# davidmilligan/MLVFS

Measured on AMD Instinct MI355X. Metric: Mpix/s, 3584x1320 14-bit unpack+badpix+cs5x5+stripes (fused, stream resident in HBM), higher is better.
Workload: dtype u16/int32

## Files before the change

### mlvfs_amd/csrc/k_frame_dev.h

```cpp
#pragma once
#include "clip.h"
#include <cstdlib>
#include <map>
#include <mutex>
#include <vector>
#include <algorithm>
#include <cstdio>
#include <type_traits>

typedef short mlv_pk16 __attribute__((ext_vector_type(2)));
__device__ __forceinline__ int mlv_min_(int a, int b) { return min(a, b); }
__device__ __forceinline__ int mlv_max_(int a, int b) { return max(a, b); }
__device__ __forceinline__ mlv_pk16 mlv_min_(mlv_pk16 a, mlv_pk16 b) { return __builtin_elementwise_min(a, b); }
__device__ __forceinline__ mlv_pk16 mlv_max_(mlv_pk16 a, mlv_pk16 b) { return __builtin_elementwise_max(a, b); }
#define MLV_NET_FN __device__ __forceinline__
#define mlv_mn(a, b) mlv_min_((a), (b))
#define mlv_mx(a, b) mlv_max_((a), (b))
#include "median_nets.h"


namespace mlv {

constexpr int TCW = FRAME_TCW;
constexpr int TCH = FRAME_TCH;
// ... 861 lines not shown
    return p;
}


template <int BPP>
__device__ __forceinline__ void item_tile_offsets(const ItemLane &L, int l_row, int w, uint32_t &pre_a, uint32_t &pre_b)
{
    constexpr uint32_t GB = (uint32_t)BPP;
    const uint32_t pitch = (uint32_t)(w >> 3) * GB;
    const uint32_t rowoff = __umul24((uint32_t)(2 * l_row), pitch) + 16u;
    pre_a = rowoff + ((uint32_t)((L.xoff_a >> 3) * (int)GB) & L.amask);
    pre_b = rowoff + ((uint32_t)((L.xoff_b >> 3) * (int)GB) & L.amask) + L.boff;
}
template <int BPP, int VEC, class LANE>
__device__ __forceinline__ void issue_tile_rows_pre(uint32_t (&r0)[4], uint32_t (&r1)[4], const uint8_t *frame, unsigned bytes, uint32_t pre_a, uint32_t pre_b,
                                                    LANE lane_of, int w, int h, int tx0, int ty0, int new0)
{
    constexpr uint32_t GB = (uint32_t)BPP;
    const uint32_t pitch = (uint32_t)(w >> 3) * GB;
    const int ybase = ty0 - 2 * HC + 2 * new0;
    uint32_t oa0, ob0, oa1, ob1, S = 0;
    if (VEC != 2 && tx0 >= 8 && tx0 + 2 * TCW + 8 <= w && ybase + 2 * TCH <= h) {
        S = (uint32_t)ybase * pitch + (uint32_t)(tx0 >> 3) * GB - 16u;
        oa0 = pre_a;
        ob0 = pre_b;
        oa1 = oa0 + pitch;
        ob1 = ob0 + pitch;
    } else {
        int l_row;
        const ItemLane L = lane_of(l_row);
        const int y = ybase + 2 * l_row;
        const int gmax = (w >> 3) - 1, g0 = tx0 >> 3;
        const uint32_t ga = __umul24((uint32_t)min(g0 + (L.xoff_a >> 3), gmax), GB);
        const uint32_t gb = __umul24((uint32_t)max(min(g0 + (L.xoff_b >> 3), gmax), 0), GB);
        const uint32_t row0 = __umul24((uint32_t)min(y, h - 1), pitch), row1 = __umul24((uint32_t)min(y + 1, h - 1), pitch);
        oa0 = (row0 + ga) & L.amask; ob0 = ((row0 + gb) & L.amask) + L.boff;
        oa1 = (row1 + ga) & L.amask; ob1 = ((row1 + gb) & L.amask) + L.boff;
        asm volatile("" : "+v"(oa0), "+v"(ob0));
    }
    const mlv_i32x4 rs = frame_rsrc(frame + S, bytes - S);
    const mlv_u32x2 a0 = mlv_rbl_x2(rs, (int)oa0, 0, AUX_DEFAULT), b0 = mlv_rbl_x2(rs, (int)ob0, 0, AUX_DEFAULT);
    const mlv_u32x2 a1 = mlv_rbl_x2(rs, (int)oa1, 0, AUX_DEFAULT), b1 = mlv_rbl_x2(rs, (int)ob1, 0, AUX_DEFAULT);
    r0[0] = a0.x; r0[1] = a0.y; r0[2] = b0.x; r0[3] = b0.y;
    r1[0] = a1.x; r1[1] = a1.y; r1[2] = b1.x; r1[3] = b1.y;
}
template <int BPP, int VEC>
__device__ __forceinline__ void issue_tile_rows(uint32_t (&r0)[4], uint32_t (&r1)[4], const uint8_t *frame, unsigned bytes, const ItemLane &L, int l_row,
                                                int w, int h, int tx0, int ty0, int new0)
{
    uint32_t pre_a, pre_b;
    item_tile_offsets<BPP>(L, l_row, w, pre_a, pre_b);
    issue_tile_rows_pre<BPP, VEC>(r0, r1, frame, bytes, pre_a, pre_b, [&](int &row) { row = l_row; return L; }, w, h, tx0, ty0, new0);
}

struct OutArgs {
    const uint2 *e2d;
    uint8_t *dst;
    size_t dst_stride;
    int stripes, coef_pk, coef_fast, white;
    int co[8];
};
__device__ __forceinline__ OutArgs out_args(KArgs kt)
{
    OutArgs o;
    o.e2d = kt->e2d; o.dst = kt->dst; o.dst_stride = kt->dst_stride;
    o.stripes = kt->stripes; o.coef_pk = kt->coef_pk; o.coef_fast = kt->coef_fast; o.white = kt->white;
#pragma unroll
    for (int i = 0; i < 8; i++) o.co[i] = kt->coef[i];
    return o;
}

__device__ __forceinline__ void put_rb(uint32_t &top, uint32_t &bot, uint32_t ur, uint32_t ub, unsigned long long m)
{
    asm("s_mov_b64 vcc, %4\n\t"
        "v_cndmask_b32_sdwa %0, %0, %2, vcc dst_sel:WORD_0 dst_unused:UNUSED_PRESERVE src0_sel:WORD_0 src1_sel:WORD_0\n\t"
        "v_cndmask_b32_sdwa %1, %1, %3, vcc dst_sel:WORD_1 dst_unused:UNUSED_PRESERVE src0_sel:WORD_1 src1_sel:WORD_0"
        : "+v"(top), "+v"(bot) : "v"(ur), "v"(ub), "s"(m) : "vcc");
}
__device__ __forceinline__ unsigned long long lanes_gt(int a, int b) { return __builtin_amdgcn_sicmp(a, b, 38); }
__device__ __forceinline__ unsigned long long lanes_ge(int a, int b) { return __builtin_amdgcn_sicmp(a, b, 39); }
__device__ __forceinline__ unsigned long long lanes_lt(int a, int b) { return __builtin_amdgcn_sicmp(a, b, 40); }

struct NoSmem {};
__device__ __forceinline__ bool smoothed_low(const int (&er)[STRIP], const int (&eb)[STRIP])
{
    const int lo = min(min(min(min(er[0], er[1]), er[2]), min(er[3], eb[0])), min(min(eb[1], eb[2]), eb[3]));
    return __any(lo < 7 * MLV_EV_RES);
}
template <int METHOD, bool PACKED, bool VECST, bool CLAMP, bool XM, bool ANYSTRIPES, bool BRIGHT, class SM, bool RAWREG = false>
__device__ __forceinline__ void strip_output_t(const SM &sm, const OutArgs &oa, int w, int h, int black, int f, int tx0, int ty0, int jj, int kk,
                                               unsigned long long msmooth, const int (&gev)[STRIP], int gev_off, const int (&er)[STRIP], const int (&eb)[STRIP], bool store,
                                               uint32_t *rtop = nullptr, uint32_t *rbot = nullptr)
{
    const int y = ty0 + 2 * jj, x = tx0 + 2 * STRIP * kk;
    uint32_t top[STRIP], bot[STRIP];
    auto read_raw = [&]() {
        if constexpr (RAWREG) {
#pragma unroll
            for (int c = 0; c < STRIP; c++) { top[c] = rtop[c]; bot[c] = rbot[c]; }
        } else {
            const uint4 v0 = *(const uint4 *)&sm.raw[2 * jj][2 * STRIP * kk];
            const uint4 v1 = *(const uint4 *)&sm.raw[2 * jj + 1][2 * STRIP * kk];
            top[0] = v0.x; top[1] = v0.y; top[2] = v0.z; top[3] = v0.w;
            bot[0] = v1.x; bot[1] = v1.y; bot[2] = v1.z; bot[3] = v1.w;
        }
    };
    if (METHOD == 0) read_raw();
    if (METHOD != 0) {
        const mlv_i32x4 rs_e2d = table_rsrc(oa.e2d, 8, E2D_RECORDS_EXT);
        int ur[STRIP], ub[STRIP], cr[STRIP], cb[STRIP];
        mlv_tab_u32x2 dr2[STRIP], db2[STRIP];
#pragma unroll
        for (int c = 0; c < STRIP; c++) {
            cr[c] = CLAMP ? min(max(er[c], 0), MLV_EV_MAX) : er[c];
            cb[c] = CLAMP ? min(max(eb[c], 0), MLV_EV_MAX) : eb[c];
            dr2[c] = mlv_sbl_x2(rs_e2d, cr[c] >> 5, 0, 0, AUX_DEFAULT);
            db2[c] = mlv_sbl_x2(rs_e2d, cb[c] >> 5, 0, 0, AUX_DEFAULT);
        }
        read_raw();
        asm volatile("" :: "v"(dr2[0]), "v"(dr2[1]), "v"(dr2[2]), "v"(dr2[3]), "v"(db2[0]), "v"(db2[1]), "v"(db2[2]), "v"(db2[3]));
#pragma unroll
        for (int c = 0; c < STRIP; c++) {
            ur[c] = (int)(__builtin_popcount(bfe_low_bits(dr2[c].y, (uint32_t)cr[c])) + dr2[c].x);
            ub[c] = (int)(__builtin_popcount(bfe_low_bits(db2[c].y, (uint32_t)cb[c])) + db2[c].x);
        }
#pragma unroll
        for (int c = 0; c < STRIP; c++) {
            unsigned long long okm = msmooth;
            if (!BRIGHT) okm &= lanes_ge((int)((uint32_t)gev[c] - (uint32_t)gev_off), 2 * MLV_EV_RES) & lanes_gt(er[c], MLV_EV_RES) & lanes_gt(eb[c], MLV_EV_RES);
            if (XM) okm &= lanes_ge(x + 2 * c, 4) & lanes_lt(x + 2 * c, w - 4);
            put_rb(top[c], bot[c], (uint32_t)ur[c], (uint32_t)ub[c], okm);
        }
    }
    if (oa.stripes) {
        const int black16 = (int)(uint16_t)black, white16 = (int)(uint16_t)oa.white;
        if (!ANYSTRIPES) stripe_strip_pk<CLAMP>(top, bot, oa.co, black16, white16);
        else if (PACKED && oa.coef_pk) stripe_strip_pk<true>(top, bot, oa.co, black16, white16);
        else if (oa.coef_fast) stripe_strip<true>(top, bot, oa.co, black16, white16);
        else stripe_strip<false>(top, bot, oa.co, black16, white16);
    }
    if constexpr (RAWREG) {
#pragma unroll
        for (int c = 0; c < STRIP; c++) { rtop[c] = top[c]; rbot[c] = bot[c]; }
    }
    if (store && y < h) {
        if (VECST) {
            if (x < w) {
                const uint32_t T = ((uint32_t)ty0 * (uint32_t)w + (uint32_t)tx0) * 2u;
                const mlv_i32x4 rs_out = frame_rsrc(oa.dst + (size_t)f * oa.dst_stride + T, (uint32_t)w * (uint32_t)h * 2u - T);
                const uint32_t vo = (__umul24((uint32_t)(2 * jj), (uint32_t)w) + 2 * STRIP * (uint32_t)kk) * 2u;
                const mlv_u32x4 vt = { top[0], top[1], top[2], top[3] }, vb = { bot[0], bot[1], bot[2], bot[3] };
                mlv_rbs_x4(vt, rs_out, (int)vo, 0, 2);
                if (y + 1 < h) mlv_rbs_x4(vb, rs_out, (int)vo, w * 2, 2);
            }
        } else {
            uint16_t *out = (uint16_t *)(oa.dst + (size_t)f * oa.dst_stride);
#pragma unroll 1
            for (int c = 0; c < STRIP; c++) {
                const int xc = x + 2 * c;
                if (xc < w) out[(size_t)y * w + xc] = (uint16_t)top[c];
                if (xc + 1 < w) out[(size_t)y * w + xc + 1] = (uint16_t)(top[c] >> 16);
                if (y + 1 < h) {
                    if (xc < w) out[(size_t)(y + 1) * w + xc] = (uint16_t)bot[c];
                    if (xc + 1 < w) out[(size_t)(y + 1) * w + xc + 1] = (uint16_t)(bot[c] >> 16);
                }
            }
        }
    }
}

template <int METHOD, bool PACKED, bool VECST, class SM>
__device__ __forceinline__ void strip_output(const SM &sm, const OutArgs &oa, int w, int h, int black, int f, int tx0, int ty0, int jj, int kk,
                                             unsigned long long msmooth, const int (&gev)[STRIP], int gev_off, const int (&er)[STRIP], const int (&eb)[STRIP], bool low_any, bool bright,
                                             bool store)
{
    const bool xm = tx0 < 4 || tx0 + 2 * TCW > w - 4;
    if (METHOD != 0 && !low_any && oa.stripes && smoothed_low(er, eb)) { low_any = true; bright = false; }
    if (oa.stripes && !(PACKED && oa.coef_pk)) {
        strip_output_t<METHOD, PACKED, VECST, true, true, true, false, SM>(sm, oa, w, h, black, f, tx0, ty0, jj, kk, msmooth, gev, gev_off, er, eb, store);
    } else if (low_any) {
// ... 35 lines not shown
```

### mlvfs_amd/csrc/k_frame_p.hip

```cpp
#include "frame_plan.h"
#include "k_stream_dev.h"

namespace mlv {

constexpr int P_WAIT_MIN = 1, P_WAIT_MAX = 15;
template <bool SPREAD_>
struct __align__(16) SmemP {
    static constexpr bool SPREAD = SPREAD_;
    uint16_t raw[2 * RH][2 * TCW];
    uint32_t pk[PH][PW];
    int ge[RH][TCW];
    uint16_t t16[MLV_T16_N + (SPREAD_ ? 64 : 0)];
    uint32_t has_patch[PMAP_WORDS];
    uint32_t xchg[3][XCHG_WORDS];
    int unc[2];
    int low[2];
    int dim[2];
    int next_tile, next_end;
    int walk[5];
    int2 carry_at[256];
    uint4 carry_spare;
};

struct PGroup {
    mlv_pk16 s[4][5];
    mlv_pk16 p0[10], p1[10];
    mlv_pk16 q[6];
};
struct PNext { mlv_pk16 s0[5], s2[5], p0[10], q[6]; };

__device__ __forceinline__ mlv_pk16 as_pk(uint32_t v) { return __builtin_bit_cast(mlv_pk16, v); }
__device__ __forceinline__ uint32_t as_u(mlv_pk16 v) { return __builtin_bit_cast(uint32_t, v); }

__device__ __forceinline__ void pchain_group(const uint32_t (*pk)[PW], int row_top, int col_left, PGroup &g)
{
    mlv_pk16 col[4][5];
#pragma unroll
    for (int r = 0; r < 5; r++) {
        const uint4 v = *(const uint4 *)&pk[row_top + r][col_left];
        col[0][r] = as_pk(v.x); col[1][r] = as_pk(v.y); col[2][r] = as_pk(v.z); col[3][r] = as_pk(v.w);
    }
#pragma unroll
    for (int c = 0; c < 4; c++) mlv_sort5(col[c], g.s[c]);
    mlv_merge55(g.s[0], g.s[1], g.p0);
    mlv_merge55(g.s[2], g.s[3], g.p1);
}
__device__ __forceinline__ void pchain_fetch_lists(const PGroup &g, PNext &n)
{
#pragma unroll
    for (int i = 0; i < 5; i++) { n.s0[i] = dpp_next(g.s[0][i]); n.s2[i] = dpp_next(g.s[2][i]); }
#pragma unroll
    for (int i = 0; i < 10; i++) n.p0[i] = dpp_next(g.p0[i]);
}
__device__ __forceinline__ void pchain_fetch_window(const PGroup &g, PNext &n)
{
#pragma unroll
    for (int i = 0; i < 6; i++) n.q[i] = dpp_next(g.q[i]);
}
__device__ __forceinline__ void pchain_publish(const PGroup &g, uint32_t *x)
{
    uint4 *o = (uint4 *)x;
    o[0] = make_uint4(as_u(g.s[0][0]), as_u(g.s[0][1]), as_u(g.s[0][2]), as_u(g.s[0][3]));
    o[1] = make_uint4(as_u(g.s[0][4]), as_u(g.s[2][0]), as_u(g.s[2][1]), as_u(g.s[2][2]));
    o[2] = make_uint4(as_u(g.s[2][3]), as_u(g.s[2][4]), as_u(g.p0[0]), as_u(g.p0[1]));
    o[3] = make_uint4(as_u(g.p0[2]), as_u(g.p0[3]), as_u(g.p0[4]), as_u(g.p0[5]));
    o[4] = make_uint4(as_u(g.p0[6]), as_u(g.p0[7]), as_u(g.p0[8]), as_u(g.p0[9]));
    o[5] = make_uint4(as_u(g.q[0]), as_u(g.q[1]), as_u(g.q[2]), as_u(g.q[3]));
    *(uint2 *)&o[6] = make_uint2(as_u(g.q[4]), as_u(g.q[5]));
}
__device__ __forceinline__ void pchain_collect_lists(const uint32_t *x, PNext &n)
{
    const uint4 *o = (const uint4 *)x;
    const uint4 a0 = o[0], a1 = o[1], a2 = o[2], a3 = o[3], a4 = o[4];
    n.s0[0] = as_pk(a0.x); n.s0[1] = as_pk(a0.y); n.s0[2] = as_pk(a0.z); n.s0[3] = as_pk(a0.w); n.s0[4] = as_pk(a1.x);
    n.s2[0] = as_pk(a1.y); n.s2[1] = as_pk(a1.z); n.s2[2] = as_pk(a1.w); n.s2[3] = as_pk(a2.x); n.s2[4] = as_pk(a2.y);
    n.p0[0] = as_pk(a2.z); n.p0[1] = as_pk(a2.w); n.p0[2] = as_pk(a3.x); n.p0[3] = as_pk(a3.y); n.p0[4] = as_pk(a3.z);
    n.p0[5] = as_pk(a3.w); n.p0[6] = as_pk(a4.x); n.p0[7] = as_pk(a4.y); n.p0[8] = as_pk(a4.z); n.p0[9] = as_pk(a4.w);
}
__device__ __forceinline__ void pchain_collect_window(const uint32_t *x, PNext &n)
{
    const uint4 a5 = *(const uint4 *)(x + 20);
    const uint2 a6 = *(const uint2 *)(x + 24);
    n.q[0] = as_pk(a5.x); n.q[1] = as_pk(a5.y); n.q[2] = as_pk(a5.z); n.q[3] = as_pk(a5.w); n.q[4] = as_pk(a6.x); n.q[5] = as_pk(a6.y);
}
__device__ __forceinline__ void pchain_finish(const PGroup &g, const PNext &n, mlv_pk16 (&o)[STRIP])
{
    mlv_pk16 q1[6], t[1];
    mlv_quad_mid6(g.p1, n.p0, q1);
    mlv_final6of11(g.q, n.s0, t);  o[0] = t[0];
    mlv_final6of11(q1, g.s[1], t); o[1] = t[0];
    mlv_final6of11(q1, n.s2, t);   o[2] = t[0];
    mlv_final6of11(n.q, g.s[3], t); o[3] = t[0];
}
__device__ __forceinline__ bool pk_uncertain(const mlv_pk16 (&o)[STRIP])
{
    typedef unsigned short upk16 __attribute__((ext_vector_type(2)));
    const upk16 off = { 32769, 32769 }, two = { 2, 2 };
    upk16 m = __builtin_bit_cast(upk16, o[0]) + off;
#pragma unroll
    for (int c = 1; c < STRIP; c++) m = __builtin_elementwise_min(m, (upk16)(__builtin_bit_cast(upk16, o[c]) + off));
    return __builtin_bit_cast(uint32_t, __builtin_elementwise_min(m, two)) != 0x00020002u;
}

__device__ __forceinline__ uint32_t add3_u32(uint32_t a, uint32_t b, uint32_t c)
{
    uint32_t r;
    asm("v_add3_u32 %0, %1, %2, %3" : "=v"(r) : "v"(a), "v"(b), "v"(c));
    return r;
}
template <int NC, bool SPREAD>
__device__ __forceinline__ void cell_multi_pk_fast(const uint32_t *p0, const uint32_t *p1, int black, const uint16_t *t, int ref_r, int ref_b,
                                                   int (&ge)[NC], uint32_t (&pk)[NC])
{
    uint32_t fb[4 * NC], tv[4 * NC];
    const float fmagic = 8388608.0f + (float)black;
#pragma unroll
    for (int c = 0; c < NC; c++) {
        const uint32_t px[4] = { p0[2 * c], p0[2 * c + 1], p1[2 * c], p1[2 * c + 1] };
#pragma unroll
        for (int i = 0; i < 4; i++) fb[4 * c + i] = __float_as_uint(__uint_as_float(px[i] | 0x4B000000u) - fmagic);
    }
#pragma unroll
    for (int i = 0; i < 4 * NC; i++) tv[i] = *(const uint16_t *)((const char *)t + t16_offset<SPREAD>(fb[i]));
    uint32_t exr[NC], exb[NC], exg[NC];
#pragma unroll
    for (int c = 0; c < NC; c++) { exr[c] = fb[4 * c] >> 8; exb[c] = fb[4 * c + 3] >> 8; exg[c] = (fb[4 * c + 1] + fb[4 * c + 2]) >> 8; }
#pragma unroll
    for (int c = 0; c < NC; c += 2) {
        asm volatile("" :: "v"(exr[c]), "v"(exb[c]), "v"(exg[c]), "v"(exr[c + 1]), "v"(exb[c + 1]), "v"(exg[c + 1]));
    }
#pragma unroll
    for (int i = 0; i < 4 * NC; i += 8) {
        asm volatile("" :: "v"(tv[i]), "v"(tv[i + 1]), "v"(tv[i + 2]), "v"(tv[i + 3]), "v"(tv[i + 4]), "v"(tv[i + 5]), "v"(tv[i + 6]), "v"(tv[i + 7]));
    }
    uint32_t nref_r = 0u - (uint32_t)ref_r, nref_b = 0u - (uint32_t)ref_b;
    asm("" : "+v"(nref_r), "+v"(nref_b));
#pragma unroll
    for (int c = 0; c < NC; c++) {
        const uint32_t gb = add3_u32(exg[c], tv[4 * c + 1], tv[4 * c + 2]) >> 1;
        ge[c] = (int)(gb - (127u << 15));
        uint32_t ngr = nref_r - gb, ngb = nref_b - gb;
        pk[c] = as_u(__builtin_amdgcn_cvt_pk_i16((int)add3_u32(exr[c], tv[4 * c + 0], ngr), (int)add3_u32(exb[c], tv[4 * c + 3], ngb)));
    }
}

template <int NC>
__device__ __forceinline__ void cell_multi_pk_tab(const uint32_t *p0, const uint32_t *p1, uint32_t koff, const int *tab, int ref_r, int ref_b,
                                                  int (&ge)[NC], uint32_t (&pk)[NC])
{
    uint32_t ev[4 * NC];
#pragma unroll
    for (int c = 0; c < NC; c++) {
        const uint32_t px[4] = { p0[2 * c], p0[2 * c + 1], p1[2 * c], p1[2 * c + 1] };
#pragma unroll
        for (int i = 0; i < 4; i++) ev[4 * c + i] = *(const uint32_t *)((const char *)tab + ((px[i] << 2) + koff));
    }
#pragma unroll
    for (int i = 0; i < 4 * NC; i += 8) {
        asm volatile("" :: "v"(ev[i]), "v"(ev[i + 1]), "v"(ev[i + 2]), "v"(ev[i + 3]), "v"(ev[i + 4]), "v"(ev[i + 5]), "v"(ev[i + 6]), "v"(ev[i + 7]));
    }
    uint32_t nref_r = 1u - (uint32_t)ref_r, nref_b = 1u - (uint32_t)ref_b;
#pragma unroll
    for (int c = 0; c < NC; c++) {
        const uint32_t gb = (ev[4 * c + 1] + ev[4 * c + 2]) >> 1;
        ge[c] = (int)gb;
        const uint32_t ng = ~gb;
        pk[c] = as_u(__builtin_amdgcn_cvt_pk_i16((int)add3_u32(ev[4 * c + 0], nref_r, ng), (int)add3_u32(ev[4 * c + 3], nref_b, ng)));
    }
}
template <int NC>
__device__ __forceinline__ void cell_multi_pk_tab_dark(const uint32_t *p0, const uint32_t *p1, uint32_t koff, const int *tab, int ref_r, int ref_b,
                                                       int (&ge)[NC], uint32_t (&pk)[NC])
{
    int ev[4 * NC];
#pragma unroll
    for (int c = 0; c < NC; c++) {
        const uint32_t px[4] = { p0[2 * c], p0[2 * c + 1], p1[2 * c], p1[2 * c + 1] };
#pragma unroll
        for (int i = 0; i < 4; i++) ev[4 * c + i] = *(const int *)((const char *)tab + max((int)((px[i] << 2) + koff), 0));
    }
#pragma unroll
    for (int i = 0; i < 4 * NC; i += 8) {
        asm volatile("" :: "v"(ev[i]), "v"(ev[i + 1]), "v"(ev[i + 2]), "v"(ev[i + 3]), "v"(ev[i + 4]), "v"(ev[i + 5]), "v"(ev[i + 6]), "v"(ev[i + 7]));
    }
// ... 413 lines not shown
    const int plane = min(max(lane - 1, 0), PARK_LANES - 1);
    const bool parks = lane >= 1 && lane <= PARK_LANES;
    for (;;) {
        const int task = stream_draw(tickets, lane);
        if (task >= ntasks) break;
        const StreamTask t = stream_task<VEC>(task, sg, segs, seg_rows, fold, S_OUT, lane, w, rows);
        const int f = t.f, c = t.c, j0 = t.j0, j1 = t.j1, nparts = t.nparts, P = t.P, roff = t.roff;
        KArgs kt = cold_args();
        const uint8_t *const frame = kt->src + (size_t)f * kt->src_stride;
        const mlv_i32x4 rs_in = frame_rsrc(frame, kt->src_bytes);
        mlv_i32x4 rs_out = { 0, 0, 0, 0 };
        int tx0 = 0;
        bool xm = false;
        uint32_t dA0[4], dA1[4], dB0[4], dB1[4];
        auto issue = [&](int r, uint32_t (&d0)[4], uint32_t (&d1)[4]) { stream_issue(rs_in, r, roff, rows, pitch, t.gbyte, d0, d1); };
        issue(j0 - 2, dA0, dA1);
        issue(j0 - 1, dB0, dB1);
        int ref_r, ref_b;
        {
            const int x0 = min(max(8 * (c * S_OUT + S_OUT / 2), 0), (w - 16) & ~1), y0 = min(j0 + j1, (h - 4) & ~1) & ~1;
            const uint32_t px = fetch_clamped<BPP>(frame, w, h, x0 + (lane & 15), y0 + (lane >> 4));
            const int ev = sm.ev[1 + min(max((int)px - black, 1), 16383)];
            constexpr int CX[5] = { 0, 3, 6, 1, 5 }, CY[5] = { 0, 0, 0, 1, 1 };
            int sdr[5], sdb[5];
#pragma unroll
            for (int k = 0; k < 5; k++) {
                const int l0 = 2 * CX[k] + 32 * CY[k];
                const int rr = __builtin_amdgcn_readlane(ev, l0), g1 = __builtin_amdgcn_readlane(ev, l0 + 1);
                const int g2 = __builtin_amdgcn_readlane(ev, l0 + 16), bb = __builtin_amdgcn_readlane(ev, l0 + 17);
                const int gg = (g1 + g2) >> 1;
                sdr[k] = rr - gg; sdb[k] = bb - gg;
            }
            auto med5 = [](const int (&v)[5]) { return med3i(v[4], max(min(v[0], v[1]), min(v[2], v[3])), min(max(v[0], v[1]), max(v[2], v[3]))); };
            ref_r = med5(sdr);
            ref_b = med5(sdb);
        }
        int n_pm = 0, pm_cell = -1;
        uint32_t pm_top = 0, pm_bot = 0;
        bool list_all = false;
        if (kt->patch) {
            KArgs ka = kt;
            const int4 *cells = ka->cells + (size_t)f * ka->n_rec;
            const int *toff = ka->tile_off;
            const int tx_n = ka->tiles_x, ty_n = ka->tiles_y;
            const int cx_lo = 4 * (c * S_OUT - 1), cx_hi = cx_lo + 4 * P;
            const int tc0 = max(cx_lo - HC, 0) / TCW, tc1 = min((cx_hi - 1 + HC) / TCW, tx_n - 1);
            for (int q = 0; q < nparts; q++) {
                const int j0q = j0 + q * seg_rows, j1q = min(j0q + seg_rows, rows);
                if (j0q >= rows) break;
                const int cy_lo = j0q - 2, cy_hi = j1q + 2;
                const int tr0 = max(cy_lo, 0) / TCH, tr1 = min((cy_hi - 1) / TCH, ty_n - 1), ntr = tr1 - tr0 + 1;
                constexpr int MAXTR = 6;
                int my_lo = 0, my_hi = 0;
                if (lane < ntr && lane < MAXTR) { my_lo = toff[(tr0 + lane) * tx_n + tc0]; my_hi = toff[(tr0 + lane) * tx_n + tc1 + 1]; }
                if (ntr > MAXTR) list_all = true;
                int4 rec[MAXTR];
#pragma unroll
                for (int i = 0; i < MAXTR; i++) {
                    const int rb = __builtin_amdgcn_readlane(my_lo, i), re = __builtin_amdgcn_readlane(my_hi, i);
                    rec[i] = (i < ntr && rb + lane < re) ? cells[rb + lane] : make_int4(-1, 0, 0, 0);
                    if (i < ntr && re - rb > 64) list_all = true;
                }
#pragma unroll
                for (int i = 0; i < MAXTR; i++) {
                    const int rcx = rec[i].x & 0xFFFF, rcy = rec[i].x >> 16;
                    const bool in = rec[i].x >= 0 && rcx >= cx_lo && rcx < cx_hi && rcy >= cy_lo && rcy < cy_hi && rcy / TCH == tr0 + i;
                    unsigned long long m = __ballot(in);
                    while (m) {
                        const int src = __builtin_ctzll(m);
                        m &= m - 1;
                        if (n_pm < 64) {
                            const int vx = __builtin_amdgcn_readlane(rec[i].x, src), vy = __builtin_amdgcn_readlane(rec[i].y, src), vz = __builtin_amdgcn_readlane(rec[i].z, src);
                            const int at = (((vx >> 16) - q * seg_rows) << 16) | (4 * P * q + (vx & 0xFFFF) - cx_lo);
                            if (lane == n_pm) { pm_cell = at; pm_top = (uint32_t)vy; pm_bot = (uint32_t)vz; }
                            n_pm++;
                        } else list_all = true;
                    }
                }
            }
        }
        uint32_t pkr[4][4] = {};
        int geA[4] = { 0, 0, 0, 0 }, geB[4] = { 0, 0, 0, 0 };
        int fl1 = 3, fl2 = 3, fl3 = 3, fl4 = 3;
        unsigned long long unc_lanes = 0;
        int unc_r0 = 1 << 30, unc_r1 = -1;
        auto load_row = [&](int r, const uint32_t (&d0)[4], const uint32_t (&d1)[4], auto after_unpack, int (&ge)[4], uint32_t (&pk)[4]) {
            uint32_t p0[8], p1[8];
            unpack8<BPP>(d0, t.sel, t.sel, t.sel, p0);
            unpack8<BPP>(d1, t.sel1, t.sel1, t.sel1, p1);
            after_unpack();
            if (n_pm) {
                unsigned long long m = __ballot(lane < n_pm && (pm_cell >> 16) == r);
                while (m) {
                    const int src = __builtin_ctzll(m);
                    m &= m - 1;
                    const int cell = __builtin_amdgcn_readlane(pm_cell, src);
                    const uint32_t t_ = (uint32_t)__builtin_amdgcn_readlane((int)pm_top, src), b_ = (uint32_t)__builtin_amdgcn_readlane((int)pm_bot, src);
                    const int cxr = cell & 0xFFFF;
                    const bool mine = (cxr >> 2) == lane;
                    const int cc = cxr & 3;
#pragma unroll
                    for (int k = 0; k < 4; k++)
                        if (mine && cc == k) { p0[2 * k] = t_ & 0xFFFFu; p0[2 * k + 1] = t_ >> 16; p1[2 * k] = b_ & 0xFFFFu; p1[2 * k + 1] = b_ >> 16; }
                }
            }
            bool dark;
            const int fl0 = stream_row_low(p0, p1, black, dark);
            if (!dark) cell_multi_pk_tab<4>(p0, p1, koff, sm.ev, ref_r, ref_b, ge, pk);
            else cell_multi_pk_tab_dark<4>(p0, p1, koff, sm.ev, ref_r, ref_b, ge, pk);
            {
                uint4 (&slot)[2][PARK_LANES] = mypark[(unsigned)(r + 2 * SLOTS) % (unsigned)SLOTS];
                if (parks) {
                    slot[0][plane] = make_uint4(p0[0] | (p0[1] << 16), p0[2] | (p0[3] << 16), p0[4] | (p0[5] << 16), p0[6] | (p0[7] << 16));
                    slot[1][plane] = make_uint4(p1[0] | (p1[1] << 16), p1[2] | (p1[3] << 16), p1[4] | (p1[5] << 16), p1[6] | (p1[7] << 16));
                }
            }
            return fl0;
        };
        auto sort_common = [&](const uint32_t (&ra)[4], const uint32_t (&rb)[4], const uint32_t (&rc)[4], const uint32_t (&rd)[4], mlv_pk16 (&c4)[4][4]) {
#pragma unroll
            for (int cc = 0; cc < 4; cc++) {
                const mlv_pk16 v[4] = { as_pk(ra[cc]), as_pk(rb[cc]), as_pk(rc[cc]), as_pk(rd[cc]) };
                mlv_sort4(v, c4[cc]);
            }
        };
        auto finish_row = [&](int jr, const mlv_pk16 (&c4)[4][4], const uint32_t (&x)[4], int fl, const int (&gej)[4], auto hook) {
            const int y = 2 * jr, yl = y + 2 * roff;
            KArgs ke = cold_args();
            const uint2 *const e2d_early = ke->e2d;
            const int stripes_early = ke->stripes;
            const unsigned long long msmooth = lanes_ge(yl, 4) & lanes_lt(yl, h - 5);
            const bool smooth_row = y + 2 * (nparts - 1) * seg_rows >= 4 && y < h - 5;
            mlv_pk16 o[STRIP] = { { 0, 0 }, { 0, 0 }, { 0, 0 }, { 0, 0 } };
            if (smooth_row) {
                PGroup gq;
#pragma unroll
                for (int cc = 0; cc < 4; cc++) {
                    const mlv_pk16 xv[1] = { as_pk(x[cc]) };
                    mlv_insert4(c4[cc], xv, gq.s[cc]);
                }
                mlv_merge55(gq.s[0], gq.s[1], gq.p0);
                mlv_merge55(gq.s[2], gq.s[3], gq.p1);
                mlv_quad_mid6(gq.p0, gq.p1, gq.q);
                PNext n;
                pchain_fetch_lists(gq, n);
                pchain_fetch_window(gq, n);
                mlv_pk16 oc[STRIP];
                pchain_finish(gq, n, oc);
                o[0] = as_pk((uint32_t)dpp_prev_i((int)as_u(oc[2]))); o[1] = as_pk((uint32_t)dpp_prev_i((int)as_u(oc[3])));
                o[2] = oc[0]; o[3] = oc[1];
                const unsigned long long um = __ballot(t.writes && pk_uncertain(o)) & msmooth;
                if (um) { unc_lanes |= um; unc_r0 = min(unc_r0, jr); unc_r1 = max(unc_r1, jr); }
            }
            int er[STRIP], eb[STRIP];
#pragma unroll
            for (int cc = 0; cc < STRIP; cc++) {
                er[cc] = wadd(wadd(gej[cc], ref_r), (int)o[cc].x);
                eb[cc] = wadd(wadd(gej[cc], ref_b), (int)o[cc].y);
            }
            uint32_t top[STRIP], bot[STRIP];
            {
                const uint4 (&slot)[2][PARK_LANES] = mypark[(unsigned)(jr + 2 * SLOTS) % (unsigned)SLOTS];
                const uint4 t4 = slot[0][plane], b4 = slot[1][plane];
                top[0] = t4.x; top[1] = t4.y; top[2] = t4.z; top[3] = t4.w;
                bot[0] = b4.x; bot[1] = b4.y; bot[2] = b4.z; bot[3] = b4.w;
            }
            OutArgs oa = out_args(cold_args());
            oa.e2d = e2d_early; oa.stripes = stripes_early;
            stream_output<5>(oa, t, tx0, xm, rs_out, w, h, black, jr, yl, msmooth, fl, gej, er, eb, top, bot, hook);
        };
        auto named_as_used = [](const uint32_t (&n0)[4], const uint32_t (&n1)[4]) {
            asm volatile("" :: "v"(n0[0]), "v"(n0[1]), "v"(n0[2]), "v"(n0[3]), "v"(n1[0]), "v"(n1[1]), "v"(n1[2]), "v"(n1[3]));
        };
        auto pair_step = [&](auto OUT, int r) {
            int ge0[4], ge1[4];
            uint32_t pk0[4], pk1[4];
            mlv_pk16 c4[4][4];
            auto early_a = [&] { if constexpr (!OUT.value) issue(r + 2, dA0, dA1); };
            auto early_b = [&] { if constexpr (!OUT.value) issue(r + 3, dB0, dB1); };
            auto late_a = [&] { named_as_used(dB0, dB1); issue(r + 2, dA0, dA1); };
            auto late_b = [&] { named_as_used(dA0, dA1); issue(r + 3, dB0, dB1); };
            const int f0 = load_row(r, dA0, dA1, early_a, ge0, pk0);
            if constexpr (OUT.value) {
                sort_common(pkr[1], pkr[2], pkr[3], pk0, c4);
                finish_row(r - 2, c4, pkr[0], f0 | fl1 | fl2 | fl3 | fl4, geA, late_a);
            }
            const int f1 = load_row(r + 1, dB0, dB1, early_b, ge1, pk1);
            if constexpr (OUT.value) finish_row(r - 1, c4, pk1, f1 | f0 | fl1 | fl2 | fl3, geB, late_b);
#pragma unroll
            for (int i = 0; i < 4; i++) { pkr[0][i] = pkr[2][i]; pkr[1][i] = pkr[3][i]; pkr[2][i] = pk0[i]; pkr[3][i] = pk1[i]; geA[i] = ge0[i]; geB[i] = ge1[i]; }
            fl4 = fl2; fl3 = fl1; fl2 = f0; fl1 = f1;
        };
        auto single_step = [&](int r, const uint32_t (&d0)[4], const uint32_t (&d1)[4]) {
            int ge0[4];
            uint32_t pk0[4];
            mlv_pk16 c4[4][4];
            const int f0 = load_row(r, d0, d1, [] {}, ge0, pk0);
            sort_common(pkr[1], pkr[2], pkr[3], pk0, c4);
            finish_row(r - 2, c4, pkr[0], f0 | fl1 | fl2 | fl3 | fl4, geA, StreamNoHook());
#pragma unroll
            for (int i = 0; i < 4; i++) { pkr[0][i] = pkr[1][i]; pkr[1][i] = pkr[2][i]; pkr[2][i] = pkr[3][i]; pkr[3][i] = pk0[i]; geA[i] = geB[i]; geB[i] = ge0[i]; }
            fl4 = fl3; fl3 = fl2; fl2 = fl1; fl1 = f0;
        };
        constexpr std::true_type Y{};
        constexpr std::false_type N{};
        int r = j0 - 2;
#pragma unroll 1
        for (; r < j0 + 2; r += 2) pair_step(N, r);
        named_as_used(dA0, dA1);
        {
            KArgs ko = cold_args();
            rs_out = frame_rsrc(ko->dst + (size_t)f * ko->dst_stride, (uint32_t)w * (uint32_t)h * 2u);
            tx0 = 8 * (c * S_OUT - 1);
            xm = c == 0 || 8 * (c * S_OUT + S_OUT) > w - 4;
        }
#pragma unroll 1
        for (; r < j1; r += 2) pair_step(Y, r);
#pragma unroll 1
        for (bool second = false; r <= j1 + 1; r++, second = true) {
            uint32_t e0[4], e1[4];
#pragma unroll
            for (int i = 0; i < 4; i++) { e0[i] = second ? dB0[i] : dA0[i]; e1[i] = second ? dB1[i] : dA1[i]; }
            single_step(r, e0, e1);
        }
        if (list_all) { unc_lanes = ~0ull; unc_r0 = j0; unc_r1 = j1 - 1; }
        if (unc_lanes && lane == 0) {
            KArgs kl = cold_args();
            const int tnx = kl->tiles_x, tny = kl->tiles_y;
            int *ctl = kl->wl_ctl;
            for (int q = 0; q < nparts; q++) {
                const unsigned long long mq = P == 64 ? unc_lanes : (unc_lanes >> (q * P)) & ((1ull << P) - 1);
                const int r0 = unc_r0 + q * seg_rows, r1 = min(unc_r1 + q * seg_rows, rows - 1);
                if (!mq || r0 >= rows) continue;
                const int l0 = __builtin_ctzll(mq), l1 = 63 - __builtin_clzll(mq);
                const int cx0 = max(4 * (c * S_OUT + l0 - 1), 0), cx1 = min(4 * (c * S_OUT + l1 - 1) + 3, w / 2 - 1);
                const int tc0 = cx0 / TCW, tc1 = min(cx1 / TCW, tnx - 1), tr0 = r0 / TCH, tr1 = min(r1 / TCH, tny - 1);
                for (int tc = tc0; tc <= tc1; tc++) {
                    const int i = atomicAdd(&ctl[0], 1);
                    kl->wl[i] = make_int2(f * tnx * tny + tc * tny + tr0, tr1 - tr0 + 1);
                    atomicAdd(&ctl[3], tr1 - tr0 + 1);
                }
            }
        }
    }
    stream_last_out(tickets, lane, WAVES, [] {});
}

void launch_frame_p(const FramePlan &pl, int method, bool packed, int vec, bool spread, hipStream_t stream, const FrameArgs &a)
{
#ifdef KFP_ONLY
    hipLaunchKernelGGL((k_frame_p<true, 1, false>), dim3(pl.first_grid), dim3(256), 0, stream, a);
#else
    with_layout(method, packed, vec, spread, [&](auto M, auto P, auto V, auto S) {
        if constexpr (M.value == 5 && P.value && (V.value == 1 || V.value == 2)) {
            if (pl.first == FirstKernel::p5) {
                hipLaunchKernelGGL((k_frame_p5<false, V.value>), dim3((pl.first_grid + 3) / 4), dim3(1024), 0, stream, a, pl.cols, pl.segs, pl.seg_rows,
                                   pl.fold, FRAME_STREAM_COLW);
                return;
            }
        }
        if constexpr (M.value == 5 && V.value != 0)
            hipLaunchKernelGGL((k_frame_p<P.value, V.value, S.value>), dim3(pl.first_grid), dim3(256), 0, stream, a);
    });
#endif
}

void preload_k_frame_p() { hipFuncAttributes fa; (void)hipFuncGetAttributes(&fa, (const void *)k_frame_p<true, 1, false>); (void)hipGetLastError(); }

}
```

### mlvfs_amd/csrc/k_frame_s.hip

```cpp
#include "frame_plan.h"
#include "k_stream_dev.h"

namespace mlv {

template <bool SPREAD, int VEC, int METHOD>
__global__ __launch_bounds__(256, 4) void k_frame_s(const FrameArgs a, int cols, int segs, int seg_rows, int fold, int S_OUT)
{
    constexpr int BPP = 14;
    __shared__ __align__(16) uint16_t t16[MLV_T16_N + (SPREAD ? 64 : 0)];
    load_t16_rel<SPREAD>(t16, a.t16, (int)threadIdx.x);
    __syncthreads();
    const int lane = (int)threadIdx.x & 63;
    const int w = a.w, h = a.h, black = a.black;
    const int rows = h >> 1;
    const StreamGrid sg = stream_grid(cols, segs, fold);
    const int ntasks = a.nframes * sg.per_frame;
    const uint32_t pitch = (uint32_t)(w >> 3) * 14u;
    const OutArgs oa = out_args(cold_args());
    int *tickets = a.tickets;
    for (;;) {
        const int task = stream_draw(tickets, lane);
        if (task >= ntasks) break;
        const StreamTask t = stream_task<VEC>(task, sg, segs, seg_rows, fold, S_OUT, lane, w, rows);
        const int f = t.f, j0 = t.j0, j1 = t.j1, roff = t.roff;
        const mlv_i32x4 rs_in = frame_rsrc(a.src + (size_t)f * a.src_stride, a.src_bytes);
        const mlv_i32x4 rs_out = frame_rsrc(oa.dst + (size_t)f * oa.dst_stride, (uint32_t)w * (uint32_t)h * 2u);
        const int tx0 = 8 * (t.c * S_OUT - 1);
        const bool xm = t.c == 0 || 8 * (t.c * S_OUT + S_OUT) > w - 4;

        uint32_t dA0[4], dA1[4], dB0[4], dB1[4];
        auto issue = [&](int r, uint32_t (&d0)[4], uint32_t (&d1)[4]) { stream_issue(rs_in, r, roff, rows, pitch, t.gbyte, d0, d1); };
        int dr2[STRIP] = { 0, 0, 0, 0 }, db2[STRIP] = { 0, 0, 0, 0 };
        int dr1[STRIP] = { 0, 0, 0, 0 }, db1[STRIP] = { 0, 0, 0, 0 }, ge1[STRIP] = { 0, 0, 0, 0 };
        uint32_t top1[STRIP] = { 0, 0, 0, 0 }, bot1[STRIP] = { 0, 0, 0, 0 };
        int flags1 = 3, flags2 = 3;
        int dark_steps = 0;
        issue(j0 - 1, dA0, dA1);
        issue(j0, dB0, dB1);
        auto step = [&](int r, uint32_t (&d0)[4], uint32_t (&d1)[4]) {
            uint32_t p0[8], p1[8];
            unpack8<BPP>(d0, t.sel, t.sel, t.sel, p0);
            unpack8<BPP>(d1, t.sel1, t.sel1, t.sel1, p1);
            if (r + 2 <= j1) issue(r + 2, d0, d1);
            bool dark;
            const int flags0 = stream_row_low(p0, p1, black, dark);
            dark_steps += dark ? 1 : 0;
            int ge[STRIP], dr[STRIP], db[STRIP];
            if (!dark) cell_multi_ev_fast<4, SPREAD>(p0, p1, black, t16, ge, dr, db);
            else {
#pragma unroll
                for (int cc = 0; cc < 4; cc += 2) {
                    int g2[2], r2[2], b2[2];
                    cell_multi_ev_dark<2, SPREAD>(p0 + 2 * cc, p1 + 2 * cc, black, t16, g2, r2, b2);
                    ge[cc] = g2[0]; ge[cc + 1] = g2[1]; dr[cc] = r2[0]; dr[cc + 1] = r2[1]; db[cc] = b2[0]; db[cc + 1] = b2[1];
                }
            }
            uint32_t top[STRIP], bot[STRIP];
#pragma unroll
            for (int cc = 0; cc < STRIP; cc++) { top[cc] = p0[2 * cc] | (p0[2 * cc + 1] << 16); bot[cc] = p1[2 * cc] | (p1[2 * cc + 1] << 16); }
            if (r - 1 >= j0) {
                const int jr = r - 1, y = 2 * jr, yl = y + 2 * roff;
                const bool smooth_row = y + 2 * (t.nparts - 1) * seg_rows >= 4 && y < h - 5;
                int er[STRIP] = { 0, 0, 0, 0 }, eb[STRIP] = { 0, 0, 0, 0 };
                if (smooth_row && METHOD == 2) {
                    const int lr = dpp_prev_i(dr1[3]), lb = dpp_prev_i(db1[3]);
                    const int rr_ = dpp_next_i(dr1[0]), rb = dpp_next_i(db1[0]);
#pragma unroll
                    for (int cc = 0; cc < STRIP; cc++) {
                        const int vr[5] = { dr2[cc], cc ? dr1[cc - 1] : lr, dr1[cc], cc < 3 ? dr1[cc + 1] : rr_, dr[cc] };
                        const int vb[5] = { db2[cc], cc ? db1[cc - 1] : lb, db1[cc], cc < 3 ? db1[cc + 1] : rb, db[cc] };
                        int o[1];
                        mlv_median5(vr, o); er[cc] = wadd(ge1[cc], o[0]);
                        mlv_median5(vb, o); eb[cc] = wadd(ge1[cc], o[0]);
                    }
                }
                if (smooth_row && METHOD == 3) {
                    auto med9 = [&](const int (&up)[STRIP], const int (&mid)[STRIP], const int (&dn)[STRIP], int (&e)[STRIP]) {
                        int lo[STRIP + 2], mi[STRIP + 2], hi[STRIP + 2];
#pragma unroll
                        for (int cc = 0; cc < STRIP; cc++) {
                            lo[cc + 1] = min(min(up[cc], mid[cc]), dn[cc]);
                            hi[cc + 1] = max(max(up[cc], mid[cc]), dn[cc]);
                            mi[cc + 1] = med3i(up[cc], mid[cc], dn[cc]);
                        }
                        lo[0] = dpp_prev_i(lo[STRIP]); mi[0] = dpp_prev_i(mi[STRIP]); hi[0] = dpp_prev_i(hi[STRIP]);
                        lo[STRIP + 1] = dpp_next_i(lo[1]); mi[STRIP + 1] = dpp_next_i(mi[1]); hi[STRIP + 1] = dpp_next_i(hi[1]);
#pragma unroll
                        for (int cc = 0; cc < STRIP; cc++)
                            e[cc] = wadd(ge1[cc], med3i(max(max(lo[cc], lo[cc + 1]), lo[cc + 2]), med3i(mi[cc], mi[cc + 1], mi[cc + 2]),
                                                         min(min(hi[cc], hi[cc + 1]), hi[cc + 2])));
                    };
                    med9(dr2, dr1, dr, er);
                    med9(db2, db1, db, eb);
                }
                const unsigned long long msmooth = lanes_ge(yl, 4) & lanes_lt(yl, h - 5);
                stream_output<METHOD>(oa, t, tx0, xm, rs_out, w, h, black, jr, yl, msmooth, flags0 | flags1 | flags2, ge1, er, eb, top1, bot1);
            }
#pragma unroll
            for (int cc = 0; cc < STRIP; cc++) {
                dr2[cc] = dr1[cc]; db2[cc] = db1[cc];
                dr1[cc] = dr[cc]; db1[cc] = db[cc]; ge1[cc] = ge[cc];
                top1[cc] = top[cc]; bot1[cc] = bot[cc];
            }
            flags2 = flags1; flags1 = flags0;
        };
        for (int r = j0 - 1; r <= j1; r += 2) {
            step(r, dA0, dA1);
            if (r + 1 <= j1) step(r + 1, dB0, dB1);
        }
        if (lane == 0 && dark_steps) atomicAdd(&a.wl_ctl[0], dark_steps);
    }
    stream_last_out(tickets, lane, 4, [&] { if (a.wl_stat) { __atomic_store_n(a.wl_stat, a.wl_ctl[0], __ATOMIC_RELAXED); __threadfence_system(); } });
}

void launch_frame_s(const FramePlan &pl, int method, int vec, bool spread, hipStream_t stream, const FrameArgs &a)
{
    with_layout(method, true, vec, spread, [&](auto M, auto P, auto V, auto S) {
        if constexpr ((M.value == 2 || M.value == 3) && P.value && (V.value == 1 || V.value == 2))
            hipLaunchKernelGGL((k_frame_s<S.value, V.value, M.value>), dim3(pl.first_grid), dim3(256), 0, stream, a, pl.cols, pl.segs, pl.seg_rows,
                               pl.fold, FRAME_STREAM_COLW);
    });
}

void preload_k_frame_s() { hipFuncAttributes fa; (void)hipFuncGetAttributes(&fa, (const void *)k_frame_s<false, 1, 2>); (void)hipGetLastError(); }

}
```

### mlvfs_amd/csrc/k_stream_dev.h

```cpp
#pragma once
#include "k_frame_dev.h"

namespace mlv {

struct StreamGrid { int ncols_full, nfolded, per_frame; };
__device__ __forceinline__ StreamGrid stream_grid(int cols, int segs, int fold)
{
    StreamGrid sg;
    sg.ncols_full = fold > 1 ? cols - 1 : cols;
    sg.nfolded = fold > 1 ? (segs + fold - 1) / fold : 0;
    sg.per_frame = sg.ncols_full * segs + sg.nfolded;
    return sg;
}

__device__ __forceinline__ int stream_draw(int *tickets, int lane)
{
    int task = 0;
    if (lane == 0) task = atomicAdd(&tickets[0], 1);
    return __builtin_amdgcn_readfirstlane(task);
}

struct StreamTask {
    int f, c;
    int j0, j1;
    int nparts, P;
    int pl, part, roff;
    int g;
    bool writes;
    uint32_t gbyte;
    uint32_t sel, sel1;
};
template <int VEC>
__device__ __forceinline__ StreamTask stream_task(int task, const StreamGrid &sg, int segs, int seg_rows, int fold, int S_OUT, int lane, int w, int rows)
{
    StreamTask t;
    const int gmax = (w >> 3) - 1;
    t.f = task / sg.per_frame;
    const int rem = task - t.f * sg.per_frame;
    const bool folded = rem >= sg.ncols_full * segs;
    t.c = folded ? sg.ncols_full : rem / segs;
    const int seg = folded ? (rem - sg.ncols_full * segs) * fold : rem - t.c * segs;
    t.j0 = seg * seg_rows; t.j1 = min(t.j0 + seg_rows, rows);
    t.nparts = folded ? fold : 1; t.P = folded ? 64 / fold : 64;
    t.pl = lane & (t.P - 1); t.part = folded ? lane / t.P : 0;
    t.roff = t.part * seg_rows;
    const int g_true = t.c * S_OUT + t.pl - 1;
    t.g = min(max(g_true, 0), gmax);
    t.writes = t.pl >= 1 && t.pl <= min(S_OUT, t.P - 2) && g_true <= gmax && t.j0 + t.roff < rows;
    t.gbyte = (uint32_t)t.g * 14u;
    t.sel = (t.g & 1) ? SEL_MIS : SEL_SWAP;
    t.sel1 = VEC == 2 ? t.sel ^ (SEL_SWAP ^ SEL_MIS) : t.sel;
    return t;
}

__device__ __forceinline__ void stream_issue(mlv_i32x4 rs_in, int r, int roff, int rows, uint32_t pitch, uint32_t gbyte, uint32_t (&d0)[4], uint32_t (&d1)[4])
{
    const int rr = min(max(r + roff, 0), rows - 1);
    const uint32_t o0u = __umul24((uint32_t)(2 * rr), pitch) + gbyte, o0 = o0u & ~3u, o1 = (o0u + pitch) & ~3u;
    const mlv_u32x2 a0 = mlv_rbl_x2(rs_in, (int)o0, 0, AUX_DEFAULT), b0 = mlv_rbl_x2(rs_in, (int)o0 + 8, 0, AUX_DEFAULT);
    const mlv_u32x2 a1 = mlv_rbl_x2(rs_in, (int)o1, 0, AUX_DEFAULT), b1 = mlv_rbl_x2(rs_in, (int)o1 + 8, 0, AUX_DEFAULT);
    d0[0] = a0.x; d0[1] = a0.y; d0[2] = b0.x; d0[3] = b0.y;
    d1[0] = a1.x; d1[1] = a1.y; d1[2] = b1.x; d1[3] = b1.y;
}

__device__ __forceinline__ int stream_row_low(const uint32_t (&p0)[8], const uint32_t (&p1)[8], int black, bool &dark)
{
    uint32_t lo = min(p0[0], p1[0]);
#pragma unroll
    for (int i = 1; i < 8; i++) lo = min(min(lo, p0[i]), p1[i]);
    dark = __any((int)lo <= black);
    int fl = 0;
    if (__any((int)lo <= black + 255)) fl = __any((int)lo <= black + 64) ? 3 : 2;
    return fl;
}

struct StreamNoHook { __device__ __forceinline__ void operator()() const {} };
template <int METHOD, class BEFORE_STORES = StreamNoHook>
__device__ __forceinline__ void stream_output(const OutArgs &oa, const StreamTask &t, int tx0, bool xm, mlv_i32x4 rs_out, int w, int h, int black, int jr, int yl,
                                              unsigned long long msmooth, int fl, const int (&ge)[STRIP], const int (&er)[STRIP], const int (&eb)[STRIP],
                                              uint32_t (&top)[STRIP], uint32_t (&bot)[STRIP], BEFORE_STORES before_stores = BEFORE_STORES())
{
    fl |= oa.stripes && smoothed_low(er, eb) ? 1 : 0;
    auto out = [&](auto CLAMP, auto XM, auto BRIGHT) {
        strip_output_t<METHOD, true, true, CLAMP.value, XM.value, false, BRIGHT.value, NoSmem, true>(NoSmem(), oa, w, h, black, t.f, tx0, 0, jr, t.pl, msmooth,
                                                                                                     ge, 0, er, eb, false, top, bot);
    };
    constexpr std::true_type Y{};
    constexpr std::false_type N{};
    if (fl & 1) { if (xm) out(Y, Y, N); else out(Y, N, N); }
    else if (xm) out(N, Y, N);
    else if (fl == 0) out(N, N, Y);
    else out(N, N, N);
    before_stores();
    if (t.writes) {
        const uint32_t vo = (__umul24((uint32_t)yl, (uint32_t)w) + (uint32_t)(8 * t.g)) * 2u;
        const mlv_u32x4 vt = { top[0], top[1], top[2], top[3] }, vb = { bot[0], bot[1], bot[2], bot[3] };
        mlv_rbs_x4(vt, rs_out, (int)vo, 0, 2);
        mlv_rbs_x4(vb, rs_out, (int)vo, w * 2, 2);
    }
}

template <class AFTER>
__device__ __forceinline__ void stream_last_out(int *tickets, int lane, int waves_per_wg, AFTER after)
{
    if (lane == 0) {
        const int nwaves = (int)gridDim.x * waves_per_wg;
        if (atomicAdd(&tickets[1], 1) == nwaves - 1) {
            tickets[0] = 0; tickets[1] = 0;
            after();
        }
    }
}

}
```

Before: 971,200.

## Defer parked raw reads, use direct lane compares, and unroll pair loop by two

The parked raw top/bottom pixels are now read from LDS through a lambda inside strip_output_t instead of before it, so they are loaded only when needed and hold registers for less time. Several __ballot calls are replaced with direct scalar compare masks (sicmp/uicmp), and the write mask is hoisted out of the loop. The stripes low-exposure check moves to the callers, using a popcount kept in an SGPR. The main pair_step loop is unrolled by two with a peeled odd step, trading code size and register pressure for fewer loop branches.

```diff
diff --git a/mlvfs_amd/csrc/k_frame_dev.h b/mlvfs_amd/csrc/k_frame_dev.h
--- a/mlvfs_amd/csrc/k_frame_dev.h
+++ b/mlvfs_amd/csrc/k_frame_dev.h
@@ -967,20 +967,22 @@
 __device__ __forceinline__ unsigned long long lanes_lt(int a, int b) { return __builtin_amdgcn_sicmp(a, b, 40); }
 
 struct NoSmem {};
+struct NoRaw {};
 __device__ __forceinline__ bool smoothed_low(const int (&er)[STRIP], const int (&eb)[STRIP])
 {
     const int lo = min(min(min(min(er[0], er[1]), er[2]), min(er[3], eb[0])), min(min(eb[1], eb[2]), eb[3]));
     return __any(lo < 7 * MLV_EV_RES);
 }
-template <int METHOD, bool PACKED, bool VECST, bool CLAMP, bool XM, bool ANYSTRIPES, bool BRIGHT, class SM, bool RAWREG = false>
+template <int METHOD, bool PACKED, bool VECST, bool CLAMP, bool XM, bool ANYSTRIPES, bool BRIGHT, class SM, bool RAWREG = false, class RAW = NoRaw>
 __device__ __forceinline__ void strip_output_t(const SM &sm, const OutArgs &oa, int w, int h, int black, int f, int tx0, int ty0, int jj, int kk,
                                                unsigned long long msmooth, const int (&gev)[STRIP], int gev_off, const int (&er)[STRIP], const int (&eb)[STRIP], bool store,
-                                               uint32_t *rtop = nullptr, uint32_t *rbot = nullptr)
+                                               uint32_t *rtop = nullptr, uint32_t *rbot = nullptr, RAW raw = RAW())
 {
     const int y = ty0 + 2 * jj, x = tx0 + 2 * STRIP * kk;
     uint32_t top[STRIP], bot[STRIP];
     auto read_raw = [&]() {
-        if constexpr (RAWREG) {
+        if constexpr (RAWREG && !std::is_same<RAW, NoRaw>::value) raw(top, bot);
+        else if constexpr (RAWREG) {
 #pragma unroll
             for (int c = 0; c < STRIP; c++) { top[c] = rtop[c]; bot[c] = rbot[c]; }
         } else {
diff --git a/mlvfs_amd/csrc/k_frame_p.hip b/mlvfs_amd/csrc/k_frame_p.hip
--- a/mlvfs_amd/csrc/k_frame_p.hip
+++ b/mlvfs_amd/csrc/k_frame_p.hip
@@ -100,6 +100,15 @@
 #pragma unroll
     for (int c = 1; c < STRIP; c++) m = __builtin_elementwise_min(m, (upk16)(__builtin_bit_cast(upk16, o[c]) + off));
     return __builtin_bit_cast(uint32_t, __builtin_elementwise_min(m, two)) != 0x00020002u;
+}
+__device__ __forceinline__ unsigned long long pk_uncertain_lanes(const mlv_pk16 (&o)[STRIP])
+{
+    typedef unsigned short upk16 __attribute__((ext_vector_type(2)));
+    const upk16 off = { 32769, 32769 }, two = { 2, 2 };
+    upk16 m = __builtin_bit_cast(upk16, o[0]) + off;
+#pragma unroll
+    for (int c = 1; c < STRIP; c++) m = __builtin_elementwise_min(m, (upk16)(__builtin_bit_cast(upk16, o[c]) + off));
+    return __builtin_amdgcn_uicmp(__builtin_bit_cast(uint32_t, __builtin_elementwise_min(m, two)), 0x00020002u, 33);
 }
 
 __device__ __forceinline__ uint32_t add3_u32(uint32_t a, uint32_t b, uint32_t c)
@@ -679,6 +688,7 @@
         uint32_t pkr[4][4] = {};
         int geA[4] = { 0, 0, 0, 0 }, geB[4] = { 0, 0, 0, 0 };
         int fl1 = 3, fl2 = 3, fl3 = 3, fl4 = 3;
+        const unsigned long long wmask = __ballot(t.writes);
         unsigned long long unc_lanes = 0;
         int unc_r0 = 1 << 30, unc_r1 = -1;
         auto load_row = [&](int r, const uint32_t (&d0)[4], const uint32_t (&d1)[4], auto after_unpack, int (&ge)[4], uint32_t (&pk)[4]) {
@@ -687,7 +697,7 @@
             unpack8<BPP>(d1, t.sel1, t.sel1, t.sel1, p1);
             after_unpack();
             if (n_pm) {
-                unsigned long long m = __ballot(lane < n_pm && (pm_cell >> 16) == r);
+                unsigned long long m = lanes_lt(lane, n_pm) & __builtin_amdgcn_sicmp(pm_cell >> 16, r, 32);
                 while (m) {
                     const int src = __builtin_ctzll(m);
                     m &= m - 1;
@@ -746,7 +756,7 @@
                 pchain_finish(gq, n, oc);
                 o[0] = as_pk((uint32_t)dpp_prev_i((int)as_u(oc[2]))); o[1] = as_pk((uint32_t)dpp_prev_i((int)as_u(oc[3])));
                 o[2] = oc[0]; o[3] = oc[1];
-                const unsigned long long um = __ballot(t.writes && pk_uncertain(o)) & msmooth;
+                const unsigned long long um = pk_uncertain_lanes(o) & wmask & msmooth;
                 if (um) { unc_lanes |= um; unc_r0 = min(unc_r0, jr); unc_r1 = max(unc_r1, jr); }
             }
             int er[STRIP], eb[STRIP];
@@ -756,15 +766,21 @@
                 eb[cc] = wadd(wadd(gej[cc], ref_b), (int)o[cc].y);
             }
             uint32_t top[STRIP], bot[STRIP];
-            {
-                const uint4 (&slot)[2][PARK_LANES] = mypark[(unsigned)(jr + 2 * SLOTS) % (unsigned)SLOTS];
-                const uint4 t4 = slot[0][plane], b4 = slot[1][plane];
-                top[0] = t4.x; top[1] = t4.y; top[2] = t4.z; top[3] = t4.w;
-                bot[0] = b4.x; bot[1] = b4.y; bot[2] = b4.z; bot[3] = b4.w;
-            }
+            const uint4 *const pslot = &mypark[(unsigned)(jr + 2 * SLOTS) % (unsigned)SLOTS][0][plane];
+            auto parked = [pslot](uint32_t (&tp)[STRIP], uint32_t (&bt)[STRIP]) {
+                const uint4 t4 = pslot[0], b4 = pslot[PARK_LANES];
+                tp[0] = t4.x; tp[1] = t4.y; tp[2] = t4.z; tp[3] = t4.w;
+                bt[0] = b4.x; bt[1] = b4.y; bt[2] = b4.z; bt[3] = b4.w;
+            };
             OutArgs oa = out_args(cold_args());
             oa.e2d = e2d_early; oa.stripes = stripes_early;
-            stream_output<5>(oa, t, tx0, xm, rs_out, w, h, black, jr, yl, msmooth, fl, gej, er, eb, top, bot, hook);
+            if (stripes_early) {
+                const int lo = min(min(min(min(er[0], er[1]), er[2]), min(er[3], eb[0])), min(min(eb[1], eb[2]), eb[3]));
+                int nlow = __builtin_popcountll(lanes_lt(lo, 7 * MLV_EV_RES));
+                asm("" : "+s"(nlow));
+                fl |= min(nlow, 1);
+            }
+            stream_output<5>(oa, t, tx0, xm, rs_out, w, h, black, jr, yl, msmooth, fl, gej, er, eb, top, bot, hook, parked);
         };
         auto named_as_used = [](const uint32_t (&n0)[4], const uint32_t (&n1)[4]) {
             asm volatile("" :: "v"(n0[0]), "v"(n0[1]), "v"(n0[2]), "v"(n0[3]), "v"(n1[0]), "v"(n1[1]), "v"(n1[2]), "v"(n1[3]));
@@ -811,8 +827,9 @@
             tx0 = 8 * (c * S_OUT - 1);
             xm = c == 0 || 8 * (c * S_OUT + S_OUT) > w - 4;
         }
+        if (((j1 - r + 1) >> 1) & 1) { pair_step(Y, r); r += 2; }
 #pragma unroll 1
-        for (; r < j1; r += 2) pair_step(Y, r);
+        for (; r < j1; r += 4) { pair_step(Y, r); pair_step(Y, r + 2); }
 #pragma unroll 1
         for (bool second = false; r <= j1 + 1; r++, second = true) {
             uint32_t e0[4], e1[4];
diff --git a/mlvfs_amd/csrc/k_frame_s.hip b/mlvfs_amd/csrc/k_frame_s.hip
--- a/mlvfs_amd/csrc/k_frame_s.hip
+++ b/mlvfs_amd/csrc/k_frame_s.hip
@@ -94,7 +94,8 @@
                     med9(db2, db1, db, eb);
                 }
                 const unsigned long long msmooth = lanes_ge(yl, 4) & lanes_lt(yl, h - 5);
-                stream_output<METHOD>(oa, t, tx0, xm, rs_out, w, h, black, jr, yl, msmooth, flags0 | flags1 | flags2, ge1, er, eb, top1, bot1);
+                stream_output<METHOD>(oa, t, tx0, xm, rs_out, w, h, black, jr, yl, msmooth, flags0 | flags1 | flags2 | (oa.stripes && smoothed_low(er, eb) ? 1 : 0),
+                                      ge1, er, eb, top1, bot1);
             }
 #pragma unroll
             for (int cc = 0; cc < STRIP; cc++) {
diff --git a/mlvfs_amd/csrc/k_stream_dev.h b/mlvfs_amd/csrc/k_stream_dev.h
--- a/mlvfs_amd/csrc/k_stream_dev.h
+++ b/mlvfs_amd/csrc/k_stream_dev.h
@@ -75,15 +75,14 @@
 }
 
 struct StreamNoHook { __device__ __forceinline__ void operator()() const {} };
-template <int METHOD, class BEFORE_STORES = StreamNoHook>
+template <int METHOD, class BEFORE_STORES = StreamNoHook, class RAW = NoRaw>
 __device__ __forceinline__ void stream_output(const OutArgs &oa, const StreamTask &t, int tx0, bool xm, mlv_i32x4 rs_out, int w, int h, int black, int jr, int yl,
                                               unsigned long long msmooth, int fl, const int (&ge)[STRIP], const int (&er)[STRIP], const int (&eb)[STRIP],
-                                              uint32_t (&top)[STRIP], uint32_t (&bot)[STRIP], BEFORE_STORES before_stores = BEFORE_STORES())
+                                              uint32_t (&top)[STRIP], uint32_t (&bot)[STRIP], BEFORE_STORES before_stores = BEFORE_STORES(), RAW raw = RAW())
 {
-    fl |= oa.stripes && smoothed_low(er, eb) ? 1 : 0;
     auto out = [&](auto CLAMP, auto XM, auto BRIGHT) {
-        strip_output_t<METHOD, true, true, CLAMP.value, XM.value, false, BRIGHT.value, NoSmem, true>(NoSmem(), oa, w, h, black, t.f, tx0, 0, jr, t.pl, msmooth,
-                                                                                                     ge, 0, er, eb, false, top, bot);
+        strip_output_t<METHOD, true, true, CLAMP.value, XM.value, false, BRIGHT.value, NoSmem, true, RAW>(NoSmem(), oa, w, h, black, t.f, tx0, 0, jr, t.pl, msmooth,
+                                                                                                          ge, 0, er, eb, false, top, bot, raw);
     };
     constexpr std::true_type Y{};
     constexpr std::false_type N{};
```

Result: faster. 983,300, median of 6 (+1.2%).
